# boiseHPSim/ldpcGpuTegra

Hardware: AMD Instinct MI355X
Metric: decoded Mbit/s + BER@SNR, DVB-S2 N=64800 r=1/2, 50 iters, 1/2/4/8 MI355X (higher is better)
Workload: dtype int8; 1 GPU; dvbs2_r1_2 layered int8 offset-min-sum (offset 1), 50 iters, batch 4096 codewords per GPU; code=dvbs2_r1_2, batch_per_gpu=4096, global_batch=4096, iters=50, kernel=coop3, parallelism=codeword shards x1 (no collective)

## Files before the change

### include/ldpc_mi355x.h

```cpp
#ifndef LDPC_MI355X_H
#define LDPC_MI355X_H

#include <stddef.h>
#include <stdint.h>

#ifdef __cplusplus
extern "C" {
#endif

#define LDPC_ABI_VERSION 1

enum {
    LDPC_OK = 0,
    LDPC_EINVAL = -1,
    LDPC_EUNSUPPORTED = -2,
    LDPC_EDEVICE = -3,
    LDPC_ENOMEM = -4,
    LDPC_EIO = -5
};

enum {
    LDPC_ALGO_OMS = 0,
    LDPC_ALGO_NMS = 1,
    LDPC_ALGO_MS = 2,
// ... 26 lines not shown
int ldpc_code_from_dvbs2_table(int n, int k_info, int n_rows, const int *row_len,
                               const int *row_addr, ldpc_code **out);
int ldpc_code_load(const char *path, ldpc_code **out);
int ldpc_code_info(const ldpc_code *h, int *n, int *m, int *e, int *n_groups, int *max_deg);
int ldpc_code_edges(const ldpc_code *h, uint32_t *edge_var, int *group_deg, int *group_cnt);
int ldpc_code_plan_info(const ldpc_code *h, int *staircase, int *n_windows, int *min_hazard);
int ldpc_code_window_plan(const ldpc_code *h, int S, int P, int *first, int *count, int max_windows,
                          int *n_windows);
int ldpc_code_coop_plan(const ldpc_code *h, int S, int R, int *first, int *count, int max_windows,
                        int *n_windows, int *tail, int *n_fwd);
int ldpc_code_coop_plan_dist(const ldpc_code *h, int S, int R, int dist, int *first, int *count, int max_windows,
                             int *n_windows, int *tail, int *n_fwd);
int ldpc_code_coop3_lc_info(const ldpc_code *h, int *slots, int *max_slots, int *residencies, int *prologue,
                            int *epilogue);
int ldpc_code_coop3_lc_banks(const ldpc_code *h, long long *swizzled, long long *plain);
int ldpc_code_layer_info(const ldpc_code *h, int *n_layers, int *max_width, int *lds_i8, int *lds_f32);
void ldpc_code_destroy(ldpc_code *h);

int ldpc_ctx_create(const ldpc_code *h, int device, int max_batch, ldpc_ctx **out);
void ldpc_ctx_destroy(ldpc_ctx *ctx);
int ldpc_ctx_stream(ldpc_ctx *ctx, void **hip_stream);
typedef enum ldpc_kernel {
    LDPC_KERNEL_AUTO = 0,
    LDPC_KERNEL_GENERIC = 1,
    LDPC_KERNEL_WINDOWED = 2,
    LDPC_KERNEL_WINDOWED2 = 3,
    LDPC_KERNEL_COOP = 5,
    LDPC_KERNEL_LDS = 7,
    LDPC_KERNEL_COOP3 = 8,
    LDPC_KERNEL_LDSEP = 9,
// ... 128 lines not shown
```

### ldpcgputegra_amd/_lib.py

```python
import ctypes as C
import os

_HERE = os.path.dirname(os.path.abspath(__file__))
LIB_PATH = os.environ.get("LDPC_MI355X_LIB") or os.path.join(_HERE, "libldpc_mi355x.so")

LDPC_OK, LDPC_EINVAL, LDPC_EUNSUPPORTED, LDPC_EDEVICE, LDPC_ENOMEM, LDPC_EIO = 0, -1, -2, -3, -4, -5
ALGO_OMS, ALGO_NMS, ALGO_MS, ALGO_BP = 0, 1, 2, 3


def source_hash():
    import hashlib
    root = os.path.dirname(_HERE)
    h = hashlib.sha256()
    for d in (os.path.join(_HERE, "csrc"), os.path.join(root, "include")):
        for f in sorted(os.listdir(d)):
            fp = os.path.join(d, f)
            if os.path.isfile(fp):
                h.update(f.encode())
                with open(fp, "rb") as fh:
                    h.update(fh.read())
    if os.path.abspath(LIB_PATH) != os.path.abspath(os.path.join(_HERE, "libldpc_mi355x.so")):
        stamp = LIB_PATH + ".defines"
        if os.path.exists(stamp):
            with open(stamp, "rb") as fh:
# ... 26 lines not shown
    "ldpc_last_error": (C.c_char_p, []),
    "ldpc_abi_version": (I, []),
    "ldpc_device_count": (I, [C.POINTER(I)]),
    "ldpc_code_create": (I, [I, I, I, P, P, P, C.POINTER(P)]),
    "ldpc_code_from_dvbs2_table": (I, [I, I, I, P, P, C.POINTER(P)]),
    "ldpc_code_load": (I, [C.c_char_p, C.POINTER(P)]),
    "ldpc_code_info": (I, [P, C.POINTER(I), C.POINTER(I), C.POINTER(I), C.POINTER(I), C.POINTER(I)]),
    "ldpc_code_edges": (I, [P, P, P, P]),
    "ldpc_code_plan_info": (I, [P, C.POINTER(I), C.POINTER(I), C.POINTER(I)]),
    "ldpc_code_layer_info": (I, [P, C.POINTER(I), C.POINTER(I), C.POINTER(I), C.POINTER(I)]),
    "ldpc_code_window_plan": (I, [P, I, I, P, P, I, C.POINTER(I)]),
    "ldpc_code_coop_plan": (I, [P, I, I, P, P, I, C.POINTER(I), C.POINTER(I), C.POINTER(I)]),
    "ldpc_code_coop_plan_dist": (I, [P, I, I, I, P, P, I, C.POINTER(I), C.POINTER(I), C.POINTER(I)]),
    "ldpc_code_coop3_lc_info": (I, [P] + [C.POINTER(I)] * 5),
    "ldpc_code_coop3_lc_banks": (I, [P, C.POINTER(C.c_longlong), C.POINTER(C.c_longlong)]),
    "ldpc_code_destroy": (None, [P]),
    "ldpc_ctx_create": (I, [P, I, I, C.POINTER(P)]),
    "ldpc_ctx_destroy": (None, [P]),
    "ldpc_ctx_stream": (I, [P, C.POINTER(P)]),
    "ldpc_ctx_set_kernel": (I, [P, I]),
    "ldpc_ctx_get_kernel": (I, [P, C.POINTER(I)]),
    "ldpc_ctx_set_bp_staircase": (I, [P, I]),
    "ldpc_ctx_get_bp_staircase": (I, [P, C.POINTER(I)]),
    "ldpc_ctx_set_f16_all_codes": (I, [P, I]),
    "ldpc_ctx_get_f16_all_codes": (I, [P, C.POINTER(I)]),
    "ldpc_ctx_set_f16_edge_parallel": (I, [P, I]),
    "ldpc_ctx_get_f16_edge_parallel": (I, [P, C.POINTER(I)]),
    "ldpc_f16_lds_shape_rule": (I, [I, I, I, I]),
    "ldpc_bp_staircase_width_model": (I, [I, I, I, C.c_uint]),
    "ldpc_ctx_last_kernel": (I, [P, C.POINTER(I)]),
# ... 114 lines not shown
```

### ldpcgputegra_amd/codes.py

```python
import ctypes as C
import os
import struct

import numpy as np

from . import _lib

CODE_DIR = os.path.join(os.path.dirname(os.path.abspath(__file__)), "codes")

ALIASES = {
    "dvbs2": "dvbs2_r1_2",
    "64800x32400": "dvbs2_r1_2",
    "64800x21600": "dvbs2_r2_3",
    "64800x7200": "dvbs2_r8_9",
    "64800x6480": "dvbs2_r9_10",
    "80211n_648": "648x324",
}


def code_path(name):
    name = ALIASES.get(name, name)
    for ext in (".ldpc", ".txt"):
        p = os.path.join(CODE_DIR, name + ext)
        if os.path.exists(p):
# ... 179 lines not shown
                                              C.byref(n), C.byref(t), C.byref(f)))
        return dict(windows=list(zip(first.tolist(), count.tolist())), tail=t.value, n_fwd=f.value)

    def coop3_line_cache(self):
        v = [C.c_int() for _ in range(5)]
        _lib.check(_lib.lib().ldpc_code_coop3_lc_info(self._h, *[C.byref(x) for x in v]))
        if v[0].value == 0:
            return None
        return dict(zip(("slots", "max_slots", "residencies", "prologue", "epilogue"), (x.value for x in v)))

    def coop3_lc_banks(self):
        a, b = C.c_longlong(), C.c_longlong()
        _lib.check(_lib.lib().ldpc_code_coop3_lc_banks(self._h, C.byref(a), C.byref(b)))
        return dict(swizzled=a.value, plain=b.value)

    def __del__(self):
        h = getattr(self, "_h", None)
        if h is not None and _lib._lib is not None:
            _lib._lib.ldpc_code_destroy(h)
            self._h = None


class Encoder:

    def __init__(self, code):
        self.code = code if isinstance(code, Code) else Code(code)
        L = _lib.lib()
        h = C.c_void_p()
        _lib.check(L.ldpc_encoder_create(self.code.handle, C.byref(h)))
        self._h = h
# ... 23 lines not shown
```

### ldpcgputegra_amd/csrc/coop.h

```cpp
#pragma once
#include "kernels.h"
#include "ldpc_internal.h"

struct CoopCode {
    int valid;
    int d0;
    int S, R;
    int nw;
    int tail;
    int n_fwd;
    int x0;
    int m0, d1;
    uint32_t *d_tab;
    int lc_slots, n_lc_pro, n_lc_epi;
    uint32_t *d_lc_pro, *d_lc_epi;
};

bool coop_params_ok(const ldpc_params *p);
int coop_upload(const ldpc_code *h, CoopCode *cc);
void coop_free(CoopCode *cc);
int launch_coop(const DecodeLaunch &L, const CoopCode &cc, hipStream_t s);
int coop_early_begin(const DecodeLaunch &L, hipStream_t s);
int coop_early_after_iter(const DecodeLaunch &L, int it, hipStream_t s);
int coop_plan_windows(const ldpc_code *h, int S, int R, int dist, std::vector<int> &first, std::vector<int> &count,
                      int *tail, int *n_fwd);

constexpr uint32_t COOP_M_ACT = 1u << 20;
// ... 8 lines not shown
    std::vector<int> first, count;
    int tail = -1, n_fwd = 0;
    std::vector<uint32_t> tab;
};
int coop_build_plan(const ldpc_code *h, int S, int R, int dist, int recw, CoopPlan &o, bool want_tab);

bool coop3_params_ok(const ldpc_params *p, const CoopCode &cc);
bool coop3_stride_ok(int stride);
void coop3_group_layout(const ldpc_code *h, size_t *vpart, size_t *block);
size_t coop3_group_bytes(const ldpc_code *h);
int coop3_mrec(int d0);
int coop3_upload(const ldpc_code *h, CoopCode *cc);
struct Coop3Host {
    CoopPlan pl;
    int S = 0, nw = 0, recw = 0, d0 = 0;
};
int coop3_plan_host(const ldpc_code *h, int ws, int r, Coop3Host &o);
struct LcPlan;
int coop3_plan_lc(const ldpc_code *h, Coop3Host &ho, LcPlan &lp);
int launch_coop3(const DecodeLaunch &L, const CoopCode &cc, hipStream_t s);
int coop3_et_stage_iters(int batch, int iters);

constexpr int LC_GAP = 10;
constexpr int LC_LEAD = 3;
constexpr int LC_PUT = 2;
constexpr int LC_SLOT_BITS = 10;
constexpr uint32_t LC_SLOT_MASK = (1u << LC_SLOT_BITS) - 1;
struct LcPlan {
    int slots = 0;
    int residencies = 0;
// ... 12 lines not shown
```

### ldpcgputegra_amd/csrc/coop3.hip

```cpp
#include "coop3_kernel.h"

using namespace c3;

namespace {

__global__ void fill_iters3_k(int batch, int32_t *iters_used, int iters)
{
    const int b = blockIdx.x * blockDim.x + threadIdx.x;
    if (b < batch) iters_used[b] = iters;
}

int env_int3(const char *name, int def)
{
    const char *e = getenv(name);
    return (e && *e) ? atoi(e) : def;
}

template <int WS>
void report_stamps3(const unsigned long long *d, int grid, hipStream_t s)
{
    constexpr int nwaves = WS + 2, CHW = Cfg<WS, 2>::CHW;
    std::vector<unsigned long long> h((size_t)grid * nwaves * 8);
    if (hipStreamSynchronize(s) != hipSuccess ||
        hipMemcpy(h.data(), d, h.size() * sizeof(h[0]), hipMemcpyDeviceToHost) != hipSuccess)
// ... 44 lines not shown
}
template <int D> struct RecwOf { static constexpr int v = G3<D>::RECW; };
template <int D> struct WsOf { static constexpr int v = G3<D>::WS; };
template <int D> struct LcsOf { static constexpr int v = G3<D>::LCS; };
template <int D> struct SmemOf { static constexpr size_t v = sizeof(Smem3<D, G3<D>::WS, 2>); };
template <int D> struct DistOf { static constexpr int v = G3<D>::DIST; };
template <int D> struct SOf { static constexpr int v = G3<D>::S; };
template <int D> struct XrOf { static constexpr int v = G3<D>::XR; };
template <int D> struct MrecOf { static constexpr int v = G3<D>::MREC; };
int g3_recw(int d0) { return g3_at<RecwOf>(d0); }
int g3_ws(int d0) { return g3_at<WsOf>(d0); }
size_t g3_smem(int d0) { return g3_at<SmemOf>(d0); }
int g3_dist(int d0) { return g3_at<DistOf>(d0); }
int g3_s(int d0) { return g3_at<SOf>(d0); }
int g3_xr(int d0) { return g3_at<XrOf>(d0); }
bool g3_degree_ok(int d0) { return d0 == 7 || d0 == 10 || d0 == 14 || d0 == 22 || d0 == 27 || d0 == 30; }
static_assert(SmemOf<7>::v + 512 <= 160 * 1024 && SmemOf<10>::v + 512 <= 160 * 1024 && SmemOf<14>::v + 512 <= 160 * 1024 &&
                  SmemOf<22>::v + 512 <= 160 * 1024 && SmemOf<27>::v + 512 <= 160 * 1024 &&
                  SmemOf<30>::v + 512 <= 160 * 1024,
              "LDS: the workgroup's Smem3 plus the ET kernel's static words fit 160 KB");
int g3_lcs(int d0) { return g3_at<LcsOf>(d0); }

int coop3_chain_prio(int d0) { return g3_ws(d0) == 6 ? 3 : 0; }

int coop3_mem_prio(int d0) { return g3_ws(d0) == 6 ? 2 : 0; }

}

int coop3_mrec(int d0) { return g3_degree_ok(d0) ? g3_at<MrecOf>(d0) : 32 * ((d0 + 7) / 8 + 1); }

// ... 20 lines not shown
    CoopPlan &pl = o.pl;
    if (coop_build_plan(h, S, r + 2, dist, RECW, pl, true) != 0) return 1;
    const int nw = (int)pl.first.size();
    auto rec_at = [&](int u, int k) { return &pl.tab[((size_t)u * S + k) * RECW]; };
    auto code_at = [&](const uint32_t *rec, int j) { return (rec[D0 + 1 + j / 2] >> (16 * (j & 1))) & 0xFFFFu; };
    std::vector<char> special((size_t)nw * S, 0);
    for (int u = 0; u < nw; u++)
        for (int k = 0; k < pl.count[u]; k++)
            for (int j = 0; j < X; j++) {
                const uint32_t f = code_at(rec_at(u, k), j);
                const int EB = coop_fwd_eb(X);
                if (dist != 1 || f == COOP_FWD_NONE || (int)(f >> (6 + EB)) != 2) continue;
                special[(size_t)u * S + k] = 1;
                special[(size_t)((u + nw - 2) % nw) * S + ((f >> EB) & 63)] = 1;
            }
    std::vector<int> check_at((size_t)nw * S);
    for (int u = 0; u < nw; u++) {
        int n = 0;
        for (int pass = 0; pass < 3; pass++)
            for (int k = 0; k < S; k++) {
                const bool act = k < pl.count[u], sp = special[(size_t)u * S + k] != 0;
                if ((pass == 0 && sp) || (pass == 1 && act && !sp) || (pass == 2 && !act)) {
                    if (pass == 0 && n >= 8) return 1;
                    check_at[(size_t)u * S + n] = k;
                    n++;
                }
            }
    }
    std::vector<uint32_t> tab(pl.tab.size());
    for (int u = 0; u < nw; u++)
        for (int kn = 0; kn < S; kn++) {
            const int k = check_at[(size_t)u * S + kn];
            const uint32_t *src = rec_at(u, k);
            uint32_t *rec = &tab[((size_t)u * S + kn) * RECW];
            std::copy(src, src + D0 + 1, rec);
            if (k >= pl.count[u]) {
                for (int j = 0; j < D0; j++) rec[j] = (uint32_t)h->n;
                rec[D0] = (uint32_t)h->m;
// ... 14 lines not shown
                    for (int j = 0; j < X; j++) {
                        const uint32_t v = rec[j];
                        if (pass == 1 && wu[v] >= 0) {
                            const int d = (u - wu[v] + nw) % nw;
                            if ((d >= 1 && d <= dist) || (d == 0 && nw > 1 && wk[v] != k))
                                return ldpc_set_error(LDPC_EINVAL, "coop3 plan: variable %u in windows %d and %d", v,
                                                      wu[v], u);
                            if (d == 2 && (k >= 8 || wk[v] >= 8))
                                return ldpc_set_error(LDPC_EINVAL, "coop3 plan: distance-2 variable %u outside slab "
                                                      "wave 0 (slots %d, %d)", v, wk[v], k);
                        }
                        wu[v] = u;
                        wk[v] = k;
                    }
                }
    }
    o.S = S;
    o.nw = nw;
    o.recw = RECW;
    o.d0 = D0;
    return 0;
}

static void coop3_records(const Coop3Host &ho, const LcPlan &lp, int k, std::vector<uint32_t> &out)
{
    const int S = ho.S, nw = ho.nw, D0 = ho.d0, X = D0 - 2, RECW = ho.recw;
    const int XR = g3_xr(D0);
    const int W_X = XR, W_O = XR + 1, W_META = XR + 2, NLD = (X + 7) / 8, W_LOP = RECW - 4 * NLD;
    out.assign((size_t)nw * S * RECW, 0);
    for (int u = 0; u < nw; u++)
        for (int kk = 0; kk < S; kk++) {
// ... 50 lines not shown
    if ((e = up(&cc->d_tab, tab)) != LDPC_OK || (e = up(&cc->d_lc_pro, lp.pro)) != LDPC_OK ||
        (e = up(&cc->d_lc_epi, lp.epi)) != LDPC_OK) {
        coop_free(cc);
        return e;
    }
    cc->valid = 1;
    cc->d0 = ho.d0;
    cc->S = ho.S;
    cc->R = 2;
    cc->nw = ho.nw;
    cc->tail = ho.pl.tail;
    cc->n_fwd = ho.pl.n_fwd;
    cc->x0 = (int)h->edge_var[h->check_start[0] + ho.d0 - 2];
    cc->m0 = h->group_cnt[0];
    cc->d1 = h->group_deg[1];
    cc->lc_slots = lp.slots;
    cc->n_lc_pro = (int)lp.pro.size();
    cc->n_lc_epi = (int)lp.epi.size();
    return LDPC_OK;
}

void coop3_group_layout_nm(int n, int m, int mrec, size_t *vpart, size_t *block)
{
    const size_t vlines = ((size_t)n + 8 + 7) / 8, mlines = ((size_t)(m + 1) * mrec + 127) / 128;
    size_t lines = vlines + mlines;
    if (lines % 2 == 0) lines++;
    *vpart = vlines * 128;
    *block = lines * 128;
}
void coop3_group_layout(const ldpc_code *h, size_t *vpart, size_t *block)
// ... 142 lines not shown
    a.iters = L.iters;
    a.batch = L.batch;
    a.iter_base = 0;
    a.fill = L.iters;
    a.batch_dev = nullptr;
    a.m0 = cc.m0;
    a.d1 = cc.d1;
    a.rmm = (uint32_t)(L.msg_max * 256 + 255) * 0x00010001u;
    const bool nms = L.algo == LDPC_ALGO_NMS;
    a.coff = nms ? 0u : (uint32_t)(L.param * 256 + 255) * 0x00010001u;
    a.offp = nms ? 0u : (uint32_t)(L.param & 0xFFFF) * 0x00010001u;
    a.nmsf = nms ? (uint32_t)(L.param & 0xFFFF) * 0x00010001u : 0u;
    a.prio = std::min(3, std::max(0, env_int3("LDPC_COOP3_PRIO", coop3_chain_prio(cc.d0))));
    a.mprio = std::min(3, std::max(0, env_int3("LDPC_COOP3_MPRIO", coop3_mem_prio(cc.d0))));
    a.slab_prio = env_int3("LDPC_COOP3_SLAB_PRIO", 2);
    const int grid = L.stride / CW;
    a.remap = (grid % 8) == 0 && env_int3("LDPC_COOP3_REMAP", 1) != 0;
    const bool stamped = env_int3("LDPC_COOP3_STAMP", 0) != 0 && !nms;
    if (stamped) {
        const size_t bytes = (size_t)grid * (g3_ws(cc.d0) + 2) * 8 * sizeof(unsigned long long);
        if (hipMalloc(&a.stamps, bytes) != hipSuccess) return -1;
        (void)hipMemsetAsync(a.stamps, 0, bytes, s);
    }
    int rc;
    auto launch_et = [&](const Coop3Args &x) -> int { return launch_any(cc.d0, x, grid, true, nms, stamped, s); };
    const int k1 = et && L.V2 && L.et2 ? coop3_et_stage_iters(L.batch, L.iters) : 0;
    if (et && k1 > 0 && !stamped) {
        const int step = std::max(1, env_int3("LDPC_COOP3_ET_STEP", 5));
        size_t vpart = 0, block = 0;
        const int mrec = coop3_mrec(cc.d0);
// ... 52 lines not shown
    return rc;
}

extern "C" int ldpc_code_coop3_lc_banks(const ldpc_code *h, long long *swizzled, long long *plain)
{
    if (!h || !swizzled || !plain) return ldpc_set_error(LDPC_EINVAL, "coop3 lc banks args");
    Coop3Host ho;
    LcPlan lp;
    const int rc = coop3_plan_lc(h, ho, lp);
    if (rc < 0) return rc;
    *swizzled = rc == 0 ? lp.bank_extra : 0;
    *plain = rc == 0 ? lp.bank_extra_plain : 0;
    return LDPC_OK;
}

extern "C" int ldpc_code_coop3_lc_info(const ldpc_code *h, int *slots, int *max_slots, int *residencies,
                                       int *prologue, int *epilogue)
{
    if (!h || !slots) return ldpc_set_error(LDPC_EINVAL, "coop3 lc info args");
    Coop3Host ho;
    LcPlan lp;
    const int rc = coop3_plan_lc(h, ho, lp);
    if (rc < 0) return rc;
    *slots = rc == 0 ? lp.slots : 0;
    if (max_slots) *max_slots = rc == 0 ? g3_lcs(ho.d0) : 0;
    if (residencies) *residencies = rc == 0 ? lp.residencies : 0;
    if (prologue) *prologue = rc == 0 ? (int)lp.pro.size() : 0;
    if (epilogue) *epilogue = rc == 0 ? (int)lp.epi.size() : 0;
    return LDPC_OK;
}
// ... 1 lines not shown
```

### ldpcgputegra_amd/csrc/coop3_kernel.h

```cpp
#pragma once
#include <algorithm>
#include <cstdio>
#include <cstdlib>
#include <type_traits>
#include <vector>

#include "coop.h"

#include "pk16.h"

__device__ i32x4 rbuf_load_v4(i32x4 rsrc, int voffset, int soffset, int aux) __asm("llvm.amdgcn.raw.buffer.load.v4i32");
__device__ void rbuf_store_v4(i32x4 v, i32x4 rsrc, int voffset, int soffset, int aux)
    __asm("llvm.amdgcn.raw.buffer.store.v4i32");

namespace c3 {

LDPC_DEV void dma16_buf(i32x4 rsrc, uint32_t voff, uint32_t lds_dst)
{
    unsigned keep;
    asm volatile("s_mov_b32 %0, m0\n\ts_mov_b32 m0, %3\n\ts_nop 0\n\tbuffer_load_dwordx4 %1, %2, 0 offen lds\n\ts_mov_b32 m0, %0"
                 : "=&s"(keep)
                 : "v"(voff), "s"(rsrc), "s"(lds_dst)
                 : "memory");
}
// ... 47 lines not shown
#ifndef LDPC_C3_PRE_CHUNK_X
#define LDPC_C3_PRE_CHUNK_X 8
#endif
#ifndef LDPC_C3_POST_CHUNK_X
#ifndef LDPC_C3_RD16
#define LDPC_C3_RD16 1
#endif
#ifndef LDPC_C3_PACK2
#define LDPC_C3_PACK2 1
#endif
#define LDPC_C3_POST_CHUNK_X 8
#endif
#ifndef LDPC_C3_POST_STAGE7
#define LDPC_C3_POST_STAGE7 1
#endif
template <int WS, int R, int SPW = 8>
struct Cfg {
    static constexpr int S = SPW * WS;
    static constexpr int KAHEAD = R + 2 + DPER;
    static constexpr int NI = R + 1;
    static constexpr int NS = R + 1 < 3 ? 3 : R + 1;
    static constexpr int U = NS;
    static constexpr int CHW = WS == 4 ? 4 : (WS >= 3 ? 3 : WS);
    static constexpr int NB = S / 8;
    static_assert(TQ >= KAHEAD + 2, "table ring: a window's records are read until its stores");
    static_assert(U % NI == 0 && U % NS == 0 && U % 3 == 0, "unroll");
};

template <int D0, int WS, int R>
struct alignas(16) Smem3 {
// ... 14 lines not shown
struct Coop3Args {
    int8_t *V;
    uint8_t *Mc;
    const uint32_t *tab;
    const uint32_t *lc_pro, *lc_epi;
    unsigned long long *stamps;
    const uint32_t *ev;
    int32_t *iters_used;
    int iters, batch, m0, d1, n_pro, n_epi;
    int iter_base, fill;
    const int *batch_dev;
    int G, nw, tail, mrows, n, m, k, x0, remap, prio, slab_prio, mprio;
    uint32_t nmsf;
    size_t gstride;
    uint32_t rmm, coff, offp;
};

template <int D0, bool LEAN = false, bool KA = G3<D0>::KEEP_AD>
struct St3 {
    static constexpr int X = D0 - 2, XL = G3<D0>::XH, NW = G3<D0>::NW;
    uint32_t c[XL + 1];
    uint32_t a[LEAN ? 1 : XL + 1];
    uint32_t mn1, mn2, sacc, mx;
    uint32_t mat[NW > 1 ? NW - 1 : 1];
    uint32_t xs;
    uint32_t ad[KA ? XL : 1];
    uint32_t v[X > 8 ? 1 : X];
};

constexpr int STEP_SHIFT = 22;
// ... 61 lines not shown
template <bool NMS>
LDPC_DEV void chain_consts(uint32_t cor, uint32_t mx, uint32_t min1, uint32_t kb, const PkK &K, uint32_t fk,
                           uint32_t offp, uint32_t &A, uint32_t &B, uint32_t &EPS, uint32_t &COV, uint32_t &L,
                           uint32_t &H)
{
    COV = pk_ashr8(cor);
    const uint32_t EM = pk_sra15(kb);
    uint32_t TV;
    if constexpr (NMS) {
        TV = nms_v(pk_min(min1, K.rmm), fk);
        EPS = pk_sub(fk ^ EM, EM);
        const uint32_t efm = pk_mul_lo(pk_ashr8(mx), EPS);
        A = pk_sub(pk_shl5(COV), efm);
        B = pk_add(A, 0x001F001Fu);
    } else {
        TV = pk_ashr8(pk_max(pk_sub(pk_min(min1, K.rmm), K.coff), 0u));
        EPS = EM | 0x00010001u;
        const uint32_t base = pk_sub(COV, pk_sub(pk_ashr8(mx) ^ EM, EM));
        A = pk_sub(base, offp);
        B = pk_add(base, offp);
    }
    L = pk_max(pk_sub(COV, TV), VNEG127);
    H = pk_min(pk_add(COV, TV), V127);
}
LDPC_DEV void chain_freeze(uint32_t fm, uint32_t vo, uint32_t &L, uint32_t &H)
{
    const uint32_t VO = pk_ashr8(vo);
    L = bfi(fm, VO, L);
    H = bfi(fm, VO, H);
}
template <bool NMS, bool ODD>
LDPC_DEV void post_finish(uint32_t xr, uint32_t mx, uint32_t mn1, uint32_t mn2, uint32_t sacc0, const PkK &K,
                          uint32_t fk, uint32_t &cx, uint32_t &ax, uint32_t &min1, uint32_t &min2, uint32_t &k1,
                          uint32_t &k2, uint32_t &e1, uint32_t &e2)
{
    cx = pk_sub_sat(xr, mx);
    ax = abs_sat(cx, K.c510);
    const uint32_t sacc = sacc0 ^ cx;
    min2 = pk_max(mn1, pk_min(ax, mn2)), min1 = pk_min(ax, mn1);
    k1 = NMS ? nms_c(pk_min(min2, K.rmm), fk)
                            : pk_max(pk_sub(pk_min(min2, K.rmm), K.coff), 0u);
    k2 = NMS ? nms_c(pk_min(min1, K.rmm), fk)
                            : pk_max(pk_sub(pk_min(min1, K.rmm), K.coff), 0u);
    signed_csts(k1, k2, sacc ^ (ODD ? SIGNS : 0u), e1, e2);
}
template <int D0, int WS, int R, bool NMS = false, bool LEAN = false, bool KA_ = G3<D0>::KEEP_AD>
struct Slab3 {
    using SM = Smem3<D0, WS, R>;
    using G = G3<D0>;
    static constexpr bool KA = KA_;
    using St = St3<D0, LEAN, KA>;
    using RecT = Rec<D0>;
    using In = PreIn<D0, KA>;
    static constexpr int S = SM::S, X = G::X, XL = G::XH;
    static constexpr int SX = G::HALF ? 14 : X;
    static constexpr int SO = G::HALF ? 15 : D0 - 1;
    static constexpr int SL = G::HALF ? 15 : X;
    static constexpr bool RD16 = LDPC_C3_RD16 && KA_ && D0 == 7;
// ... 2 lines not shown
    SM &sm;
    const Coop3Args &a;
    int k, kl, q, w, lane, tail;
    uint32_t usel;
    PkK K;
    uint32_t fk;
    char *Vg;
    uint32_t lrd, lwr;
    uint32_t mrd, prd;
    uint32_t m1rd;
    uint32_t fm = 0;
    uint32_t psel = 0x0c0c0705u;
    uint32_t psel_raw = 0x0c0c0705u;
    static constexpr bool FZ_REREAD = X > 8;
    uint32_t h = 0, hm = 0, mbrd = 0;

    LDPC_DEV const char *lcb() const { return (const char *)&sm.lc[0][0]; }
    LDPC_DEV char *lcw() const { return (char *)&sm.lc[0][0]; }

    LDPC_DEV RecT read_rec(int g) const
    {
        RecT o;
        if constexpr (G::HALF) {
            const uint32_t *rw = &sm.tab[g & (TQ - 1)][k][0];
            const uint2 *e2 = (const uint2 *)(rw + XL * h);
#pragma unroll
            for (int i = 0; i < XL / 2; i++) {
                const uint2 d = e2[i];
                o.e[2 * i] = d.x;
                o.e[2 * i + 1] = d.y;
// ... 35 lines not shown
#else
            const uint2 mm = *(const uint2 *)(inb + mrd);
#endif
            in.ma[0] = mm.x;
            in.mb = mm.y;
#pragma unroll
            for (int i = 1; i < G::NMA; i++) in.ma[i] = *(const uint32_t *)(inb + m1rd + 256 * (i - 1));
        }
        in.meta = rc.w(G::W_META);
        in.wx = rc.w(G::W_X);
        in.wo = rc.w(G::W_O);
    }
    LDPC_DEV uint2 read_x_raw(int g, const St &s) const
    {
        const unsigned short *xs = (const unsigned short *)&sm.xo[g & 1][0][0] + s.xs + 16 * q;
        return make_uint2(xs[0], xs[8]);
    }
    LDPC_DEV static uint32_t x_of(uint2 x) { return perm(x.y, x.x, 0x040d000du); }
    LDPC_DEV uint32_t read_x(int g, const St &s) const
    {
        const unsigned short *xs = (const unsigned short *)&sm.xo[g & 1][0][0] + s.xs + 16 * q;
#ifdef C3X_BANK_X
        const unsigned short *xz = (const unsigned short *)&sm.xo[g & 1][0][0] + 2 * lane;
        const uint32_t x0 = xz[0], x1 = xz[1];
#else
        const uint32_t x0 = xs[0], x1 = xs[8];
#endif
        return perm(x1, x0, 0x040d000du);
    }

    LDPC_DEV static uint32_t swap1(uint32_t x) { return (uint32_t)__builtin_amdgcn_mov_dpp((int)x, 0xB1, 0xF, 0xF, true); }
    LDPC_DEV static void merge(uint32_t &min1, uint32_t &min2, uint32_t &sacc)
    {
        const uint32_t m1p = swap1(min1), m2p = swap1(min2), sp = swap1(sacc);
        min2 = pk_min(pk_max(min1, m1p), pk_min(min2, m2p));
        min1 = pk_min(min1, m1p);
        sacc ^= sp;
    }

    template <bool TL, bool FZ_ = false, int MP = -1>
    LDPC_DEV void pre(int g, const In &in, St &s) const
    {
        constexpr bool FZ = FZ_;
        const uint32_t meta = in.meta;
        uint32_t v[XL + 1];
#pragma unroll
        for (int j = 0; j <= XL; j++) v[j] = unpack_v(in.v[j], RD16 && j < XL ? USEL16 : usel);
        if constexpr (KA) {
#pragma unroll
            for (int j = 0; j < XL; j++) s.ad[j] = in.ad[j];
        }
        auto sink = [&](auto jc, uint32_t c) __attribute__((always_inline)) -> uint32_t {
            constexpr int J = decltype(jc)::value;
            if constexpr (G::HALF && J < XL && J >= X - XL) return bfi(hm, R127, c);
            else return c;
// ... 70 lines not shown
            uint32_t avl[LEAN ? XL + 1 : 1];
            auto av = [&](int j) __attribute__((always_inline)) -> uint32_t & { return LEAN ? avl[LEAN ? j : 0] : s.a[LEAN ? 0 : j]; };
            auto tail_edge = [&](auto jc, auto csc) __attribute__((always_inline)) {
                constexpr int J = decltype(jc)::value, CS = decltype(csc)::value;
                const uint32_t c = sink(jc, pk_max(pk_sub_sat(v[J], old_msg2<CS>(in.ma, t, K)), neg127));
                const uint32_t aj = sink(jc, NMS ? abs_r(c, c510) : abs_r(pk_min(c, K.rmm), c510));
                s.c[J] = c;
                av(J) = aj;
                sacc ^= c;
                min_track<2>(min1, min2, aj);
            };
            static_for<0, XL>([&](auto jc) __attribute__((always_inline)) { tail_edge(jc, jc); });
            if constexpr (G::HALF) merge(min1, min2, sacc);
            tail_edge(std::integral_constant<int, XL>{}, std::integral_constant<int, SL>{});
            const uint32_t k1 = NMS ? nms_c(pk_min(min2, K.rmm), fk)
                                    : pk_min(pk_max(pk_sub(min2, K.coff), 0u), K.rmm) & HIBYTES;
            const uint32_t k2 = NMS ? nms_c(pk_min(min1, K.rmm), fk)
                                    : pk_min(pk_max(pk_sub(min1, K.coff), 0u), K.rmm) & HIBYTES;
            uint32_t e1, e2, MAn[G::NW];
#pragma unroll
            for (int i = 0; i < G::NW; i++) MAn[i] = 0;
            signed_csts(k1, k2, sacc ^ (((D0 - 1) & 1) ? SIGNS : 0u), e1, e2);
            auto tail_new = [&](auto jc, auto csc) __attribute__((always_inline)) {
                constexpr int J = decltype(jc)::value, CS = decltype(csc)::value;
                s.c[J] = new_v_later<CS & 7>(s.c[J], av(J), min1, e1, e2, MAn[CS >> 3], neg127);
                if constexpr (FZ) s.c[J] = bfi(fm, v[J], s.c[J]);
            };
            static_for<0, XL>([&](auto jc) __attribute__((always_inline)) { tail_new(jc, jc); });
            tail_new(std::integral_constant<int, XL>{}, std::integral_constant<int, SL>{});
            s.mx = 0;
            s.sacc = 0;
            s.mn1 = MAn[0];
#pragma unroll
            for (int i = 1; i < G::NW; i++) s.mat[i - 1] = MAn[i];
            s.mn2 = perm(e2, e1, 0x07030501u);
            const uint32_t Y = pk_ashr8(s.c[XL]);
            A = B = COV = L = H = Y;
            if constexpr (NMS) {
                A = pk_shl5(Y);
                B = pk_add(A, 0x001F001Fu);
            }
            EPS = 0;
        }
        if (!(meta & COOP_M_ACT)) {
            A = COV = 0;
            B = NMS ? 0x001F001Fu : 0u;
            EPS = NMS ? 0x00200020u : 0x00010001u;
            L = VNEG127;
            H = V127;
        }
        const int cb = g & 1;
        s.xs = in.wx >> 16;
        uint4 r0, r1;
        r0.x = perm(B, A, 0x05040100u);
        r1.x = perm(B, A, 0x07060302u);
        r0.y = perm(COV, EPS, 0x05040100u);
        r1.y = perm(COV, EPS, 0x07060302u);
        r0.z = perm(H, L, 0x05040100u);
        r1.z = perm(H, L, 0x07060302u);
        r0.w = r1.w = 0;
        uint4 *cp = (uint4 *)((char *)&sm.cst[cb][0][0][q] + (in.wo >> 16));
        if (!G::HALF || h == 0) {
            cp[0] = r0;
            cp[NP] = r1;
        }
// ... 799 lines not shown
                    PkK{opaque(RNEG127), opaque(R0), opaque(C510), opaque(a.rmm), opaque(a.coff), opaque(0x03000300u),
                        opaque(0x040c000cu)},
                    opaque(a.nmsf),
                    Vg,
                    (uint32_t)(4 * (sq >> 1)),
                    (uint32_t)(2 * sq),
                    GG::HALF ? (uint32_t)(((4 * (lane & 1) + (sq >> 1)) * 8 + skl) * 16 + (sq & 1) * 8)
                             : (uint32_t)(((sq >> 1) * 8 + skl) * 16 + (sq & 1) * 8),
                    (uint32_t)((8 * GG::MP + skl) * 16 + 4 * (sq >> 1)),
                    (uint32_t)(((4 + (sq >> 2)) * 8 + skl) * 16 + (sq & 3) * 4)};
    if constexpr (GG::HALF) {
        sl.h = (uint32_t)(lane & 1);
        sl.hm = (lane & 1) ? 0xFFFFFFFFu : 0u;
        sl.mbrd = (uint32_t)(((8 + (sq >> 2)) * 8 + skl) * 16 + (sq & 3) * 4);
    }
    auto next = [&](int &u) __attribute__((always_inline)) { u = (u + 1 == a.nw) ? 0 : u + 1; };
    for (int it = 0;; it++) {
        if (STAMP) tseg = stamp3();
        {
            constexpr int PB = 12;
            for (int i0 = st_id; i0 < 8 * a.n_pro; i0 += PB * NSL) {
                uint32_t pw[PB];
                uint4 d[PB];
#pragma unroll
                for (int j = 0; j < PB; j++) pw[j] = a.lc_pro[min(i0 + j * NSL, 8 * a.n_pro - 1) >> 3];
#pragma unroll
                for (int j = 0; j < PB; j++)
                    d[j] = *(const uint4 *)(Vg + (size_t)(pw[j] & 0xFFFFu) * 128 + (uint32_t)((i0 + j * NSL) & 7) * 16u);
#pragma unroll
                for (int j = 0; j < PB; j++)
// ... 36 lines not shown
                begin(p, tx);
            }
            const bool dpo = p >= 1 && p <= G, dpr = p + 1 < G;
            const bool fast = !GU && uA != a.tail && uB != a.tail;
            PreIn<D0, KA> in;
            St3<D0, LEAN, KA> &sp = st[(s + NS - 1) % NS], &sn = st[(s + 1) % NS];
            unsigned long long t1 = 0, t2 = 0, t3 = 0;
            const bool stag = LDPC_C3_STAGGER && WS == 6 && wave > CHW;
            const bool prefirst = fast && (GG::DIST == 2 || stag);
            if (prefirst) {
                if (stag && fair) __builtin_amdgcn_s_setprio(P0);
                uint2 xe = make_uint2(0, 0);
                if (LDPC_C3_XEARLY) xe = sl.read_x_raw(p - 1, sp);
                sl.read_pre((s + 1) % NI, KA ? rcn : sl.read_rec(p + 1), in);
                if constexpr (KA) rcn = sl.read_rec(p + 2);
                sl.template pre<false, ET>(p + 1, in, sn);
                if (STAMP) t1 = stampL();
                if (stag && fair) __builtin_amdgcn_s_setprio(P1);
                const uint32_t xr = LDPC_C3_XEARLY ? Slab3<D0, WS, R, NMS, LEAN, KA>::x_of(xe) : sl.read_x(p - 1, sp);
                if (STAMP) {
                    asm volatile("" ::"v"(xr));
                    t2 = stampL();
                }
                sl.template post<false, ET>(p - 1, xr, sp);
                if (STAMP) t3 = stampL();
            } else if (fast) {
                if (fair) __builtin_amdgcn_s_setprio(P0);
                {
                    const uint32_t xr = sl.read_x(p - 1, sp);
                    if (STAMP) {
                        asm volatile("" ::"v"(xr));
                        t2 = stampL();
                    }
                    sl.template post<false, ET, MP1>(p - 1, xr, sp);
                    if (SL3::RD16 && fair) __builtin_amdgcn_s_setprio(P1);
                    sl.read_pre((s + 1) % NI, KA ? rcn : sl.read_rec(p + 1), in);
                }
                if constexpr (KA) rcn = sl.read_rec(p + 2);
                if (STAMP) t1 = stampL();
                if (!SL3::RD16 && fair) __builtin_amdgcn_s_setprio(P1);
                sl.template pre<false, ET, MP2>(p + 1, in, sn);
                if (STAMP) t3 = stampL();
            } else {
                if (dpo) {
                    const uint32_t xr = sl.read_x(p - 1, sp);
                    if (uA == a.tail)
                        sl.template post<true, ET>(p - 1, xr, sp);
                    else
                        sl.template post<false, ET>(p - 1, xr, sp);
                }
                if (STAMP) t1 = t2 = t3 = stampL();
                if (dpr) sl.read_pre((s + 1) % NI, KA ? rcn : sl.read_rec(p + 1), in);
                if constexpr (KA) rcn = sl.read_rec(p + 2);
                if (dpr) {
                    if (uB == a.tail)
                        sl.template pre<true, ET>(p + 1, in, sn);
// ... 95 lines not shown
```

### ldpcgputegra_amd/csrc/pk16.h

```cpp
#pragma once
#include <type_traits>

#include "kernels_common.h"

typedef int i32x4 __attribute__((ext_vector_type(4)));
typedef int i32x2 __attribute__((ext_vector_type(2)));

__device__ uint32_t sbuf_load_u32(i32x4 rsrc, int index, int offset, int soffset, int aux)
    __asm("llvm.amdgcn.struct.buffer.load.i32");
__device__ void sbuf_store_u16(unsigned short v, i32x4 rsrc, int index, int offset, int soffset, int aux)
    __asm("llvm.amdgcn.struct.buffer.store.i16");
__device__ i32x2 sbuf_load_v2(i32x4 rsrc, int index, int offset, int soffset, int aux)
    __asm("llvm.amdgcn.struct.buffer.load.v2i32");
__device__ void sbuf_store_v2(i32x2 v, i32x4 rsrc, int index, int offset, int soffset, int aux)
    __asm("llvm.amdgcn.struct.buffer.store.v2i32");

namespace {

constexpr int CW = 16;
constexpr int NP = 8;
constexpr int MREC = 64;

typedef short s16x2 __attribute__((ext_vector_type(2)));
typedef unsigned short u16x2 __attribute__((ext_vector_type(2)));
// ... 4 lines not shown
    i32x4 r;
    r.x = __builtin_amdgcn_readfirstlane((int)(uint32_t)a);
    r.y = __builtin_amdgcn_readfirstlane((int)((uint32_t)(a >> 32) | (stride << 16)));
    r.z = __builtin_amdgcn_readfirstlane((int)records);
    r.w = 0x00020000;
    return r;
}

LDPC_DEV s16x2 sv(uint32_t x) { return __builtin_bit_cast(s16x2, x); }
LDPC_DEV uint32_t us(s16x2 x) { return __builtin_bit_cast(uint32_t, x); }
LDPC_DEV uint32_t pk_sub_sat(uint32_t a, uint32_t b) { return us(__builtin_elementwise_sub_sat(sv(a), sv(b))); }
LDPC_DEV uint32_t pk_add_sat(uint32_t a, uint32_t b) { return us(__builtin_elementwise_add_sat(sv(a), sv(b))); }
LDPC_DEV uint32_t pk_max(uint32_t a, uint32_t b) { return us(__builtin_elementwise_max(sv(a), sv(b))); }
LDPC_DEV uint32_t pk_min(uint32_t a, uint32_t b) { return us(__builtin_elementwise_min(sv(a), sv(b))); }
LDPC_DEV uint32_t pk_sub(uint32_t a, uint32_t b) { return us(sv(a) - sv(b)); }
LDPC_DEV uint32_t pk_sra15(uint32_t a) { return us(sv(a) >> (short)15); }
LDPC_DEV uint32_t pk_mul_lo(uint32_t a, uint32_t b)
{
    return us(__builtin_bit_cast(s16x2, __builtin_bit_cast(u16x2, a) * __builtin_bit_cast(u16x2, b)));
}
LDPC_DEV uint32_t bfi(uint32_t m, uint32_t a, uint32_t b) { return (m & a) | (~m & b); }
LDPC_DEV uint32_t perm(uint32_t s0, uint32_t s1, uint32_t sel) { return __builtin_amdgcn_perm(s0, s1, sel); }
LDPC_DEV uint32_t opaque(uint32_t x)
{
    asm volatile("" : "+v"(x));
    return x;
}
LDPC_DEV int hi8(uint32_t x, int h) { return __builtin_amdgcn_sbfe((int)x, 8 + 16 * h, 8); }

constexpr uint32_t RNEG127 = 0x81FF81FFu;
// ... 111 lines not shown
```

Before: 8358 Mbit/s.

## Add pass-through slot mask and fuse saturating subtracts in coop3 pre stage

Replaces max(sub(a,b),0) with a packed unsigned saturating subtract, and computes the EPS sign flip with a packed multiply instead of xor/sub. Adds a host-computed per-wave pass-through mask so waves whose slots are never inactive skip the inactive-slot fixup in the steady-state pre stage, with a host validation check. Also adds an optional 16-bit x read path (off by default) and a new API to query slot activity. The unsigned saturation is only equivalent when the first operand is non-negative, and a wrong mask would silently skip required fixups.

```diff
diff --git a/include/ldpc_mi355x.h b/include/ldpc_mi355x.h
--- a/include/ldpc_mi355x.h
+++ b/include/ldpc_mi355x.h
@@ -64,6 +64,8 @@
 int ldpc_code_coop3_lc_info(const ldpc_code *h, int *slots, int *max_slots, int *residencies, int *prologue,
                             int *epilogue);
 int ldpc_code_coop3_lc_banks(const ldpc_code *h, long long *swizzled, long long *plain);
+int ldpc_code_coop3_slots(const ldpc_code *h, int *n_windows, int *S, int *slots_per_wave, int *tail,
+                          unsigned *pt_mask, unsigned char *active, int max_slots);
 int ldpc_code_layer_info(const ldpc_code *h, int *n_layers, int *max_width, int *lds_i8, int *lds_f32);
 void ldpc_code_destroy(ldpc_code *h);
 
diff --git a/ldpcgputegra_amd/_lib.py b/ldpcgputegra_amd/_lib.py
--- a/ldpcgputegra_amd/_lib.py
+++ b/ldpcgputegra_amd/_lib.py
@@ -64,6 +64,7 @@
     "ldpc_code_coop_plan_dist": (I, [P, I, I, I, P, P, I, C.POINTER(I), C.POINTER(I), C.POINTER(I)]),
     "ldpc_code_coop3_lc_info": (I, [P] + [C.POINTER(I)] * 5),
     "ldpc_code_coop3_lc_banks": (I, [P, C.POINTER(C.c_longlong), C.POINTER(C.c_longlong)]),
+    "ldpc_code_coop3_slots": (I, [P] + [C.POINTER(I)] * 4 + [C.POINTER(C.c_uint), P, I]),
     "ldpc_code_destroy": (None, [P]),
     "ldpc_ctx_create": (I, [P, I, I, C.POINTER(P)]),
     "ldpc_ctx_destroy": (None, [P]),
diff --git a/ldpcgputegra_amd/codes.py b/ldpcgputegra_amd/codes.py
--- a/ldpcgputegra_amd/codes.py
+++ b/ldpcgputegra_amd/codes.py
@@ -217,6 +217,18 @@
         _lib.check(_lib.lib().ldpc_code_coop3_lc_banks(self._h, C.byref(a), C.byref(b)))
         return dict(swizzled=a.value, plain=b.value)
 
+    def coop3_slots(self):
+        L = _lib.lib()
+        v = [C.c_int() for _ in range(4)]
+        m = C.c_uint()
+        _lib.check(L.ldpc_code_coop3_slots(self._h, *[C.byref(x) for x in v], C.byref(m), None, 0))
+        nw, S, spw, tail = (x.value for x in v)
+        if nw == 0:
+            return None
+        act = np.zeros((nw, S), dtype=np.uint8)
+        _lib.check(L.ldpc_code_coop3_slots(self._h, *[C.byref(x) for x in v], C.byref(m), act.ctypes.data, act.size))
+        return dict(windows=nw, S=S, slots_per_wave=spw, tail=tail, pt_mask=m.value, active=act)
+
     def __del__(self):
         h = getattr(self, "_h", None)
         if h is not None and _lib._lib is not None:
diff --git a/ldpcgputegra_amd/csrc/coop.h b/ldpcgputegra_amd/csrc/coop.h
--- a/ldpcgputegra_amd/csrc/coop.h
+++ b/ldpcgputegra_amd/csrc/coop.h
@@ -11,6 +11,7 @@
     int n_fwd;
     int x0;
     int m0, d1;
+    uint32_t pt_mask;
     uint32_t *d_tab;
     int lc_slots, n_lc_pro, n_lc_epi;
     uint32_t *d_lc_pro, *d_lc_epi;
@@ -49,6 +50,8 @@
 struct Coop3Host {
     CoopPlan pl;
     int S = 0, nw = 0, recw = 0, d0 = 0;
+    uint32_t pt_mask = 0;
+    int spw = 0;
 };
 int coop3_plan_host(const ldpc_code *h, int ws, int r, Coop3Host &o);
 struct LcPlan;
diff --git a/ldpcgputegra_amd/csrc/coop3.hip b/ldpcgputegra_amd/csrc/coop3.hip
--- a/ldpcgputegra_amd/csrc/coop3.hip
+++ b/ldpcgputegra_amd/csrc/coop3.hip
@@ -82,6 +82,8 @@
 int g3_dist(int d0) { return g3_at<DistOf>(d0); }
 int g3_s(int d0) { return g3_at<SOf>(d0); }
 int g3_xr(int d0) { return g3_at<XrOf>(d0); }
+template <int D> struct SpwOf { static constexpr int v = G3<D>::SPW; };
+int g3_spw(int d0) { return g3_at<SpwOf>(d0); }
 bool g3_degree_ok(int d0) { return d0 == 7 || d0 == 10 || d0 == 14 || d0 == 22 || d0 == 27 || d0 == 30; }
 static_assert(SmemOf<7>::v + 512 <= 160 * 1024 && SmemOf<10>::v + 512 <= 160 * 1024 && SmemOf<14>::v + 512 <= 160 * 1024 &&
                   SmemOf<22>::v + 512 <= 160 * 1024 && SmemOf<27>::v + 512 <= 160 * 1024 &&
@@ -132,7 +134,9 @@
                 special[(size_t)u * S + k] = 1;
                 special[(size_t)((u + nw - 2) % nw) * S + ((f >> EB) & 63)] = 1;
             }
+    const int spw = g3_spw(D0);
     std::vector<int> check_at((size_t)nw * S);
+    uint32_t pt_mask = 0;
     for (int u = 0; u < nw; u++) {
         int n = 0;
         for (int pass = 0; pass < 3; pass++)
@@ -140,6 +144,7 @@
                 const bool act = k < pl.count[u], sp = special[(size_t)u * S + k] != 0;
                 if ((pass == 0 && sp) || (pass == 1 && act && !sp) || (pass == 2 && !act)) {
                     if (pass == 0 && n >= 8) return 1;
+                    if (pass == 2 && u != pl.tail) pt_mask |= 1u << (n / spw);
                     check_at[(size_t)u * S + n] = k;
                     n++;
                 }
@@ -184,7 +189,14 @@
                         wk[v] = k;
                     }
                 }
-    }
+        for (int u = 0; u < nw; u++)
+            for (int k = 0; k < S && u != pl.tail; k++)
+                if (!(pl.tab[((size_t)u * S + k) * RECW + D0] & COOP_M_ACT) && !((pt_mask >> (k / spw)) & 1u))
+                    return ldpc_set_error(LDPC_EINVAL, "coop3 plan: inactive slot %d of window %d outside the "
+                                          "pass-through mask 0x%x", k, u, pt_mask);
+    }
+    o.pt_mask = pt_mask;
+    o.spw = spw;
     o.S = S;
     o.nw = nw;
     o.recw = RECW;
@@ -265,6 +277,7 @@
     cc->x0 = (int)h->edge_var[h->check_start[0] + ho.d0 - 2];
     cc->m0 = h->group_cnt[0];
     cc->d1 = h->group_deg[1];
+    cc->pt_mask = ho.pt_mask;
     cc->lc_slots = lp.slots;
     cc->n_lc_pro = (int)lp.pro.size();
     cc->n_lc_epi = (int)lp.epi.size();
@@ -437,6 +450,7 @@
     a.prio = std::min(3, std::max(0, env_int3("LDPC_COOP3_PRIO", coop3_chain_prio(cc.d0))));
     a.mprio = std::min(3, std::max(0, env_int3("LDPC_COOP3_MPRIO", coop3_mem_prio(cc.d0))));
     a.slab_prio = env_int3("LDPC_COOP3_SLAB_PRIO", 2);
+    a.pt_mask = env_int3("LDPC_COOP3_PT_ALL", 0) != 0 ? 0xFFFFFFFFu : cc.pt_mask;
     const int grid = L.stride / CW;
     a.remap = (grid % 8) == 0 && env_int3("LDPC_COOP3_REMAP", 1) != 0;
     const bool stamped = env_int3("LDPC_COOP3_STAMP", 0) != 0 && !nms;
@@ -519,6 +533,28 @@
     return LDPC_OK;
 }
 
+extern "C" int ldpc_code_coop3_slots(const ldpc_code *h, int *n_windows, int *S, int *slots_per_wave, int *tail,
+                                     unsigned *pt_mask, unsigned char *active, int max_slots)
+{
+    if (!h || !n_windows || !S || !slots_per_wave || !tail || !pt_mask)
+        return ldpc_set_error(LDPC_EINVAL, "coop3 slots args");
+    Coop3Host ho;
+    LcPlan lp;
+    const int rc = coop3_plan_lc(h, ho, lp);
+    if (rc < 0) return rc;
+    *n_windows = rc == 0 ? ho.nw : 0;
+    *S = rc == 0 ? ho.S : 0;
+    *slots_per_wave = rc == 0 ? ho.spw : 0;
+    *tail = rc == 0 ? ho.pl.tail : -1;
+    *pt_mask = rc == 0 ? ho.pt_mask : 0u;
+    if (rc == 0 && active) {
+        if (max_slots < ho.nw * ho.S) return ldpc_set_error(LDPC_EINVAL, "coop3 slots: room for %d", ho.nw * ho.S);
+        for (int i = 0; i < ho.nw * ho.S; i++)
+            active[i] = (ho.pl.tab[(size_t)i * ho.recw + ho.d0] & COOP_M_ACT) ? 1 : 0;
+    }
+    return LDPC_OK;
+}
+
 extern "C" int ldpc_code_coop3_lc_info(const ldpc_code *h, int *slots, int *max_slots, int *residencies,
                                        int *prologue, int *epilogue)
 {
diff --git a/ldpcgputegra_amd/csrc/coop3_kernel.h b/ldpcgputegra_amd/csrc/coop3_kernel.h
--- a/ldpcgputegra_amd/csrc/coop3_kernel.h
+++ b/ldpcgputegra_amd/csrc/coop3_kernel.h
@@ -85,6 +85,15 @@
 #ifndef LDPC_C3_POST_STAGE7
 #define LDPC_C3_POST_STAGE7 1
 #endif
+#ifndef LDPC_C3_EPS_MUL
+#define LDPC_C3_EPS_MUL 1
+#endif
+#ifndef LDPC_C3_PT_MASK
+#define LDPC_C3_PT_MASK 1
+#endif
+#ifndef LDPC_C3_XD16
+#define LDPC_C3_XD16 0
+#endif
 template <int WS, int R, int SPW = 8>
 struct Cfg {
     static constexpr int S = SPW * WS;
@@ -129,6 +138,7 @@
     uint32_t nmsf;
     size_t gstride;
     uint32_t rmm, coff, offp;
+    uint32_t pt_mask;
 };
 
 template <int D0, bool LEAN = false, bool KA = G3<D0>::KEEP_AD>
@@ -220,11 +230,19 @@
         A = pk_sub(pk_shl5(COV), efm);
         B = pk_add(A, 0x001F001Fu);
     } else {
-        TV = pk_ashr8(pk_max(pk_sub(pk_min(min1, K.rmm), K.coff), 0u));
+        TV = pk_ashr8(pk_subu_sat(pk_min(min1, K.rmm), K.coff));
         EPS = EM | 0x00010001u;
+#if LDPC_C3_EPS_MUL
+        const uint32_t base = pk_sub(COV, pk_mul_lo(pk_ashr8(mx), EPS));
+#else
         const uint32_t base = pk_sub(COV, pk_sub(pk_ashr8(mx) ^ EM, EM));
+#endif
+        const uint32_t lo = pk_sub(COV, TV), hi = pk_add(COV, TV);
         A = pk_sub(base, offp);
         B = pk_add(base, offp);
+        L = pk_max(lo, VNEG127);
+        H = pk_min(hi, V127);
+        return;
     }
     L = pk_max(pk_sub(COV, TV), VNEG127);
     H = pk_min(pk_add(COV, TV), V127);
@@ -245,9 +263,9 @@
     const uint32_t sacc = sacc0 ^ cx;
     min2 = pk_max(mn1, pk_min(ax, mn2)), min1 = pk_min(ax, mn1);
     k1 = NMS ? nms_c(pk_min(min2, K.rmm), fk)
-                            : pk_max(pk_sub(pk_min(min2, K.rmm), K.coff), 0u);
+                            : pk_subu_sat(pk_min(min2, K.rmm), K.coff);
     k2 = NMS ? nms_c(pk_min(min1, K.rmm), fk)
-                            : pk_max(pk_sub(pk_min(min1, K.rmm), K.coff), 0u);
+                            : pk_subu_sat(pk_min(min1, K.rmm), K.coff);
     signed_csts(k1, k2, sacc ^ (ODD ? SIGNS : 0u), e1, e2);
 }
 template <int D0, int WS, int R, bool NMS = false, bool LEAN = false, bool KA_ = G3<D0>::KEEP_AD>
@@ -280,6 +298,7 @@
     uint32_t psel_raw = 0x0c0c0705u;
     static constexpr bool FZ_REREAD = X > 8;
     uint32_t h = 0, hm = 0, mbrd = 0;
+    bool ptw = true;
 
     LDPC_DEV const char *lcb() const { return (const char *)&sm.lc[0][0]; }
     LDPC_DEV char *lcw() const { return (char *)&sm.lc[0][0]; }
@@ -345,9 +364,20 @@
     LDPC_DEV uint2 read_x_raw(int g, const St &s) const
     {
         const unsigned short *xs = (const unsigned short *)&sm.xo[g & 1][0][0] + s.xs + 16 * q;
+#if LDPC_C3_XD16
+        u16x2 v;
+        v.x = xs[0];
+        v.y = xs[8];
+        return make_uint2(__builtin_bit_cast(uint32_t, v), 0u);
+#else
         return make_uint2(xs[0], xs[8]);
-    }
+#endif
+    }
+#if LDPC_C3_XD16
+    LDPC_DEV static uint32_t x_of(uint2 x) { return perm(x.x, x.x, 0x020d000du); }
+#else
     LDPC_DEV static uint32_t x_of(uint2 x) { return perm(x.y, x.x, 0x040d000du); }
+#endif
     LDPC_DEV uint32_t read_x(int g, const St &s) const
     {
         const unsigned short *xs = (const unsigned short *)&sm.xo[g & 1][0][0] + s.xs + 16 * q;
@@ -369,7 +399,7 @@
         sacc ^= sp;
     }
 
-    template <bool TL, bool FZ_ = false, int MP = -1>
+    template <bool TL, bool FZ_ = false, int MP = -1, bool PTM = false>
     LDPC_DEV void pre(int g, const In &in, St &s) const
     {
         constexpr bool FZ = FZ_;
@@ -470,9 +500,9 @@
             if constexpr (G::HALF) merge(min1, min2, sacc);
             tail_edge(std::integral_constant<int, XL>{}, std::integral_constant<int, SL>{});
             const uint32_t k1 = NMS ? nms_c(pk_min(min2, K.rmm), fk)
-                                    : pk_min(pk_max(pk_sub(min2, K.coff), 0u), K.rmm) & HIBYTES;
+                                    : pk_min(pk_subu_sat(min2, K.coff), K.rmm) & HIBYTES;
             const uint32_t k2 = NMS ? nms_c(pk_min(min1, K.rmm), fk)
-                                    : pk_min(pk_max(pk_sub(min1, K.coff), 0u), K.rmm) & HIBYTES;
+                                    : pk_min(pk_subu_sat(min1, K.coff), K.rmm) & HIBYTES;
             uint32_t e1, e2, MAn[G::NW];
 #pragma unroll
             for (int i = 0; i < G::NW; i++) MAn[i] = 0;
@@ -498,13 +528,22 @@
             }
             EPS = 0;
         }
-        if (!(meta & COOP_M_ACT)) {
-            A = COV = 0;
-            B = NMS ? 0x001F001Fu : 0u;
-            EPS = NMS ? 0x00200020u : 0x00010001u;
-            L = VNEG127;
-            H = V127;
-        }
+        auto pass_through = [&]() __attribute__((always_inline)) {
+            if (!(meta & COOP_M_ACT)) {
+                A = COV = 0;
+                B = NMS ? 0x001F001Fu : 0u;
+                EPS = NMS ? 0x00200020u : 0x00010001u;
+                L = VNEG127;
+                H = V127;
+            }
+        };
+        if constexpr (PTM && LDPC_C3_PT_MASK) {
+            if (ptw) {
+                asm volatile("");
+                pass_through();
+            }
+        } else
+            pass_through();
         const int cb = g & 1;
         s.xs = in.wx >> 16;
         uint4 r0, r1;
@@ -1334,6 +1373,7 @@
         sl.hm = (lane & 1) ? 0xFFFFFFFFu : 0u;
         sl.mbrd = (uint32_t)(((8 + (sq >> 2)) * 8 + skl) * 16 + (sq & 3) * 4);
     }
+    sl.ptw = ((a.pt_mask >> sw) & 1u) != 0;
     auto next = [&](int &u) __attribute__((always_inline)) { u = (u + 1 == a.nw) ? 0 : u + 1; };
     for (int it = 0;; it++) {
         if (STAMP) tseg = stamp3();
@@ -1400,7 +1440,7 @@
                 if (LDPC_C3_XEARLY) xe = sl.read_x_raw(p - 1, sp);
                 sl.read_pre((s + 1) % NI, KA ? rcn : sl.read_rec(p + 1), in);
                 if constexpr (KA) rcn = sl.read_rec(p + 2);
-                sl.template pre<false, ET>(p + 1, in, sn);
+                sl.template pre<false, ET, -1, true>(p + 1, in, sn);
                 if (STAMP) t1 = stampL();
                 if (stag && fair) __builtin_amdgcn_s_setprio(P1);
                 const uint32_t xr = LDPC_C3_XEARLY ? Slab3<D0, WS, R, NMS, LEAN, KA>::x_of(xe) : sl.read_x(p - 1, sp);
@@ -1425,7 +1465,7 @@
                 if constexpr (KA) rcn = sl.read_rec(p + 2);
                 if (STAMP) t1 = stampL();
                 if (!SL3::RD16 && fair) __builtin_amdgcn_s_setprio(P1);
-                sl.template pre<false, ET, MP2>(p + 1, in, sn);
+                sl.template pre<false, ET, MP2, true>(p + 1, in, sn);
                 if (STAMP) t3 = stampL();
             } else {
                 if (dpo) {
diff --git a/ldpcgputegra_amd/csrc/pk16.h b/ldpcgputegra_amd/csrc/pk16.h
--- a/ldpcgputegra_amd/csrc/pk16.h
+++ b/ldpcgputegra_amd/csrc/pk16.h
@@ -42,6 +42,19 @@
 LDPC_DEV uint32_t pk_max(uint32_t a, uint32_t b) { return us(__builtin_elementwise_max(sv(a), sv(b))); }
 LDPC_DEV uint32_t pk_min(uint32_t a, uint32_t b) { return us(__builtin_elementwise_min(sv(a), sv(b))); }
 LDPC_DEV uint32_t pk_sub(uint32_t a, uint32_t b) { return us(sv(a) - sv(b)); }
+#ifndef LDPC_C3_SUBU_SAT
+#define LDPC_C3_SUBU_SAT 1
+#endif
+constexpr uint32_t PK_COFF_MAX = 63u * 256u + 255u;
+static_assert(PK_COFF_MAX <= 0x7FFFu, "pk_subu_sat == max(a - b, 0) needs coff's halves non-negative as i16");
+LDPC_DEV uint32_t pk_subu_sat(uint32_t a, uint32_t b)
+{
+#if LDPC_C3_SUBU_SAT
+    return __builtin_bit_cast(uint32_t, __builtin_elementwise_sub_sat(__builtin_bit_cast(u16x2, a), __builtin_bit_cast(u16x2, b)));
+#else
+    return pk_max(pk_sub(a, b), 0u);
+#endif
+}
 LDPC_DEV uint32_t pk_sra15(uint32_t a) { return us(sv(a) >> (short)15); }
 LDPC_DEV uint32_t pk_mul_lo(uint32_t a, uint32_t b)
 {
```

Measured after the change: 8471 Mbit/s (median of 6 runs). 1.4% higher.
